# AcherStyx/SSD-Object-Detection

Hardware: AMD Instinct MI355X
Metric: images/sec SSD300 train step, batch 64 (higher is better)
Workload: dtype bf16; 1 GPU; BASELINE configs[2]: SSD300 full train step (anchor match+encode, image normalisation, conv fwd, loss, conv bwd, per-variable clip (64 variables) + Adam), per-GPU batch 64, 80 classes, synthetic COCO-shaped boxes; per_gpu_batch=64, global_batch=64, parallelism=single

## Files before the change

### include/ssd_hip.h

```cpp
#ifndef SSD_HIP_H
#define SSD_HIP_H

#include <stddef.h>
#include <stdint.h>

#ifdef __cplusplus
extern "C" {
#endif

typedef enum {
    SSD_OK = 0,
    SSD_ERR_ASSERT = -1,
    SSD_ERR_VALUE = -2,
    SSD_ERR_WORKSPACE = -3,
    SSD_ERR_LAUNCH = -4,
    SSD_ERR_UNSUPPORTED = -5
} ssd_status;

typedef enum { SSD_F32 = 0, SSD_BF16 = 1 } ssd_dtype;

int ssd_hip_abi_version(void);
const char* ssd_status_string(int status);

int ssd_priors_count(const int* grid_hw, int levels, const int* ratio_off);
// ... 271 lines not shown
    SSD_PLAN_DMA_256_256, SSD_PLAN_DMA_256_128, SSD_PLAN_DMA_256_64, SSD_PLAN_DMA_128_64, SSD_PLAN_DMA_128_128,
    SSD_PLAN_CONV0_FWD, SSD_PLAN_P512, SSD_PLAN_PW,
    SSD_PLAN_WG_FIRST = 32, SSD_PLAN_WG_PATCH_16x16, SSD_PLAN_WG_PATCH_6x40, SSD_PLAN_WG_PATCH_10x24, SSD_PLAN_WG_TILE,
    SSD_PLAN_WG_GENERIC,
    SSD_PLAN_F_FLAT = 0x100,
    SSD_PLAN_F_ROWFLAT = 0x200,
    SSD_PLAN_F_SPLITK = 0x400,
    SSD_PLAN_F_POOL_FUSED = 0x800,
    SSD_PLAN_F_S2 = 0x1000,
    SSD_PLAN_F_REDUCE_WIDE = 0x2000
};
int ssd_conv2d_fwd_plan(int B, int H, int W, int Cin, int Cout, int ksize, int stride, int pad_t, int pad_l, int Ho, int Wo,
                        int pool, size_t ws_bytes);
int ssd_conv2d_head_fwd_plan(int B, int H, int W, int Cin, int per_cell, int classes, size_t ws_bytes);
int ssd_conv2d_bwd_data_plan(int B, int H, int W, int Cin, int Cout_pad, int ksize, int stride, int pad_t, int pad_l, int Ho,
                             int Wo, int accumulate, size_t ws_bytes);
int ssd_conv2d_bwd_weight_plan(int B, int H, int W, int Cin, int Cout, int ldy, int ksize, int stride, int pad_t, int pad_l,
                               int Ho, int Wo);
const char* ssd_conv_plan_name(int plan);
int ssd_conv2d_fwd_workgroups(int B, int H, int W, int Cin, int Cout, int ksize, int stride, int pad_t, int pad_l, int Ho,
                              int Wo, int pool, size_t ws_bytes);
int ssd_conv2d_bwd_data_workgroups(int B, int H, int W, int Cin, int Cout_pad, int ksize, int stride, int pad_t, int pad_l,
                                   int Ho, int Wo, int accumulate, size_t ws_bytes);

int ssd_dev_knob(const char* name, int value);

int ssd_dev_mfma_calibration_workgroups(void);
double ssd_dev_mfma_calibration_flops(int iters);
int ssd_dev_mfma_calibration(int iters, void* stamps, void* sink, void* stream);

#ifdef __cplusplus
}
#endif
#endif
```

### ssd-object-detection_amd/csrc/conv.hip

```cpp
#include <atomic>
#include <cstdint>
#include <type_traits>
#include "common.h"
#include <hip/hip_bf16.h>
#include <stdlib.h>

#include "conv_common.h"
namespace {

template <int EPI>
__global__ void k_igemm_finalize(ConvGeom g, Epilogue ep) {
    const int n4 = (g.N + 3) >> 2;
    const long long idx = (long long)blockIdx.x * blockDim.x + threadIdx.x;
    if (idx >= (long long)g.M * n4) return;
    const int m = (int)(idx / n4), n = (int)(idx - (long long)m * n4) * 4;
    const bool full = n + 3 < g.N;
    float v[4] = {0.f, 0.f, 0.f, 0.f};
    if (full && !(g.N & 3)) {
        for (int z = 0; z < ep.ksplit; ++z) {
            const float4 t = *reinterpret_cast<const float4*>(ep.slab + ((long long)z * g.M + m) * g.N + n);
            v[0] += t.x; v[1] += t.y; v[2] += t.z; v[3] += t.w;
        }
    } else {
        for (int z = 0; z < ep.ksplit; ++z) {
// ... 390 lines not shown
        asm volatile("s_waitcnt vmcnt(6)" ::: "memory");
        SSD_PHASE_MMA(1, 0, fw0)
    }
#undef SSD_PHASE_MMA
    if (wr == 0) __builtin_amdgcn_s_barrier();

    if (staged_ok<EPI>(g, ep) && !(g.ablate & 8)) {
        asm volatile("s_waitcnt vmcnt(0)" ::: "memory");
        auto row_to_m = [&](int row) { const int m = m0 + row; return m < g.M ? m : -1; };
        staged_epilogue<EPI, 256, 256, 4, 8, 512>(acc, smem, g, ep, n0, wr * 128, wc * 64, tid, row_to_m);
        return;
    }
    int mrow[8];
#pragma unroll
    for (int p = 0; p < 8; ++p) {
        const int m = m0 + wr * 128 + p * 16 + (lane & 15);
        mrow[p] = m < g.M ? m : -1;
    }
    conv_epilogue_rows<EPI, 4, 8>(acc, g, ep, mrow, n0 + wc * 64, lane);
}

constexpr int P32_PITCH = 96;
constexpr int P32_PATCH = 32 * 1024;

template <int BN, int EPI, bool FLAT>
__global__ __launch_bounds__(512) __attribute__((amdgpu_waves_per_eu(4, 4))) void k_conv3x3_patch32(
    const bf16_raw* __restrict__ x, const bf16_raw* __restrict__ w, ConvGeom g, Epilogue ep, int tiles_x, int tiles_y, int nblocks, int rowflat) {
    constexpr int CT = BN / 32;
    constexpr int PT = 4;
    constexpr int WBYTES = BN * 64;
    constexpr int OFF_W = 2 * P32_PATCH;
    constexpr int OFF_DUMMY = OFF_W + 2 * WBYTES;
    extern __shared__ __attribute__((aligned(16))) char smem[];

    const int tid = threadIdx.x, lane = tid & 63;
    const int wave = __builtin_amdgcn_readfirstlane(tid >> 6);
    const int wave_m = wave & 3, wave_n = wave >> 2;
    const int ntn = (g.N + BN - 1) / BN;
    const int kx = blockIdx.x >> 3;
    const int pblock = (kx / ntn) * 8 + (blockIdx.x & 7);
    if (pblock >= nblocks) return;
    const int n0 = (kx % ntn) * BN;
    constexpr bool flat = FLAT;
    const int Q = FLAT ? g.W + 1 : PATCH_W;
    const int img = (g.H + 1) * Q;
    int b = 0, y0 = 0, x0 = 0, f0 = 0;
// ... 162 lines not shown
                    acc[c][p] = __builtin_amdgcn_mfma_f32_16x16x32_bf16(fw[c], fx[p], acc[c][p], 0, 0, 0);
            __builtin_amdgcn_s_setprio(3);
        }
    }
    }
    if (staged_ok<EPI>(g, ep) && !(g.ablate & 8)) {
        auto row_to_m = [&](int row) {
            if (flat) return flat_pixel(f0 + row);
            const int ir = image_row(row >> 4), xx = x0 + (row & 15);
            return (ir >= 0 && xx < g.Wo) ? ir * g.Wo + xx : -1;
        };
        auto pool_index = [&](int py, int px) -> long long {
            if (flat) return -1;
            int bb = b, gy = (y0 >> 1) + py;
            const int gx = (x0 >> 1) + px;
            if (rowflat) {
                const int R = y0 + 2 * py;
                bb = fdiv(R, g.d_h1);
                gy = (R - bb * g.d_h1.d) >> 1;
                if (bb >= g.B) return -1;
            }
            return (gy < ep.pool_h && gx < ep.pool_w) ? ((long long)bb * ep.pool_h + gy) * ep.pool_w + gx : -1;
        };
        staged_epilogue<EPI, 256, BN, CT, PT, 512>(acc, smem, g, ep, n0, wave_m * 64, wave_n * (16 * CT), tid, row_to_m, pool_index);
        return;
    }
    int mrow[PT];
#pragma unroll
    for (int p = 0; p < PT; ++p) {
        if (flat) {
            mrow[p] = flat_pixel(f0 + (4 * wave_m + p) * 16 + (lane & 15));
        } else {
            const int ir = image_row(4 * wave_m + p), xx = x0 + (lane & 15);
            mrow[p] = (ir >= 0 && xx < g.Wo) ? ir * g.Wo + xx : -1;
        }
    }
    conv_epilogue_rows<EPI, CT, PT>(acc, g, ep, mrow, n0 + wave_n * (16 * CT), lane);
}

constexpr int P5_PIX = 34 * PATCH_W;
constexpr int P5_NDMA = (P5_PIX * 6 + 63) / 64;
constexpr int P5_PATCH = P5_NDMA * 1024;
constexpr int P5_WSLOT = 128 * 64;
constexpr int P5_OFF_W = 2 * P5_PATCH;
constexpr int P5_OFF_DUMMY = P5_OFF_W + 4 * P5_WSLOT;
constexpr int P5_LDS = P5_OFF_DUMMY + 1024;

template <int EPI, bool FLAT>
__global__ __launch_bounds__(512) void k_conv3x3_p512(const bf16_raw* __restrict__ x, const bf16_raw* __restrict__ w, ConvGeom g,
                                                      Epilogue ep, int tiles_x, int tiles_y, int nblocks, int rowflat) {
    constexpr int BN = 128, CT = 4, PT = 8;
    extern __shared__ __attribute__((aligned(16))) char smem[];
    const int tid = threadIdx.x, lane = tid & 63;
    const int wave = __builtin_amdgcn_readfirstlane(tid >> 6);
    const int wave_m = wave & 3, wave_n = wave >> 2;
    const int ntn = (g.N + BN - 1) / BN;
    const int kx = blockIdx.x >> 3;
    const int pblock = (kx / ntn) * 8 + (blockIdx.x & 7);
    if (pblock >= nblocks) return;
    const int n0 = (kx % ntn) * BN;
    const int Q = FLAT ? g.W + 1 : PATCH_W;
    const int img = (g.H + 1) * Q;
    int b = 0, y0 = 0, x0 = 0, f0 = 0;
    if constexpr (FLAT) {
        f0 = pblock * 512;
    } else {
        int t = pblock;
        const int tx = t % tiles_x; t /= tiles_x;
        x0 = tx * 16;
// ... 58 lines not shown
    for (int c = 0; c < CT; ++c)
#pragma unroll
        for (int p = 0; p < PT; ++p) acc[c][p] = f32x4_t{0.f, 0.f, 0.f, 0.f};

    const int frow = lane & 15, fk = lane >> 4;
    const int xbase = (FLAT ? 8 * wave_m * 16 + frow : 8 * wave_m * PATCH_W + frow) * P32_PITCH + fk * 16;
    constexpr int prow = (FLAT ? 16 : PATCH_W) * P32_PITCH;
    int wbase;
    {
        const int row = wave_n * 64 + frow;
        wbase = P5_OFF_W + row * 64 + ((fk ^ ((-(row >> 2)) & 3)) << 4);
    }
    auto ldf = [&](int addr) { return lds_read_b128_scoped(smem + addr, smem); };
    auto load_x = [&](bf16x8_t (&fx)[PT], int pb, int tap) {
        const int tapoff = pb + xbase + ((tap / 3) * Q + tap % 3) * P32_PITCH;
#pragma unroll
        for (int p = 0; p < PT; ++p) fx[p] = ldf(tapoff + p * prow);
    };
    auto load_w = [&](bf16x8_t (&fw)[CT], int step) {
        const int wb = (step & 3) * P5_WSLOT;
#pragma unroll
        for (int c = 0; c < CT; ++c) fw[c] = ldf(wb + wbase + c * 1024);
    };
#pragma unroll
    for (int j = 0; j < 8; ++j) dma_piece(0, 0, j, true);
    dma_w(0); dma_w(1); dma_w(2);
    bf16x8_t fxa[PT], fxb[PT], fwa[CT], fwb[CT];
    asm volatile("s_waitcnt vmcnt(2)" ::: "memory");
    __builtin_amdgcn_s_barrier();
    load_x(fxa, 0, 0);
    load_w(fwa, 0);
    auto run_chunk = [&](int chunk, auto par_tag) {
        constexpr int PAR = decltype(par_tag)::value;
        const int pb = (chunk & 1) * P5_PATCH;
        const bool next_chunk = chunk + 1 < nchunk && !(g.ablate & 32);
#pragma unroll
        for (int tap = 0; tap < 9; ++tap) {
            constexpr int NT[9] = {1, 3, 5, 5, 5, 3, 1, 1, 1};
            if (NT[tap] == 1) asm volatile("s_waitcnt vmcnt(1) lgkmcnt(0)" ::: "memory");
            else if (NT[tap] == 3) asm volatile("s_waitcnt vmcnt(3) lgkmcnt(0)" ::: "memory");
            else asm volatile("s_waitcnt vmcnt(5) lgkmcnt(0)" ::: "memory");
            __builtin_amdgcn_s_barrier();
            const int step = chunk * 9 + tap;
            dma_w(step + 3);
            if (tap < 4) {
                dma_piece(chunk + 1, (chunk + 1) & 1, 2 * tap, next_chunk);
// ... 5 lines not shown
            bf16x8_t (&fwn)[CT] = ((tap + PAR) & 1) ? fwa : fwb;
            if (tap < 8) load_x(fxn, pb, tap + 1);
            else load_x(fxn, next_chunk ? (P5_PATCH - pb) : pb, next_chunk ? 0 : 8);
            load_w(fwn, step + 1 < nstep ? step + 1 : step);
#pragma unroll
            for (int c = 0; c < CT; ++c)
#pragma unroll
                for (int p = 0; p < PT; ++p)
                    acc[c][p] = __builtin_amdgcn_mfma_f32_16x16x32_bf16(fwc[c], fxc[p], acc[c][p], 0, 0, 0);
#define SSD_P5_GROUP(NM_) __builtin_amdgcn_sched_group_barrier(0x008, NM_, 0); __builtin_amdgcn_sched_group_barrier(0x100, 1, 0)
            SSD_P5_GROUP(2); SSD_P5_GROUP(2); SSD_P5_GROUP(2); SSD_P5_GROUP(2); SSD_P5_GROUP(2); SSD_P5_GROUP(2);
            SSD_P5_GROUP(2); SSD_P5_GROUP(2); SSD_P5_GROUP(2); SSD_P5_GROUP(2); SSD_P5_GROUP(2); SSD_P5_GROUP(2);
            __builtin_amdgcn_sched_group_barrier(0x008, 8, 0);
#undef SSD_P5_GROUP
            __builtin_amdgcn_sched_barrier(0);
        }
    };
    for (int chunk = 0; chunk < nchunk; chunk += 2) {
        run_chunk(chunk, std::integral_constant<int, 0>{});
        run_chunk(chunk + 1, std::integral_constant<int, 1>{});
    }
    asm volatile("s_waitcnt vmcnt(0) lgkmcnt(0)" ::: "memory");
    if (staged_ok<EPI>(g, ep)) {
        auto row_to_m = [&](int row) {
            if constexpr (FLAT) return flat_pixel(f0 + row);
            const int ir = image_row(row >> 4), xx = x0 + (row & 15);
            return (ir >= 0 && xx < g.Wo) ? ir * g.Wo + xx : -1;
        };
        auto pool_index = [&](int py, int px) -> long long {
            if (FLAT) return -1;
            int bb = b, gy = (y0 >> 1) + py;
            const int gx = (x0 >> 1) + px;
            if (rowflat) {
                const int R = y0 + 2 * py;
                bb = fdiv(R, g.d_h1);
                gy = (R - bb * g.d_h1.d) >> 1;
                if (bb >= g.B) return -1;
            }
            return (gy < ep.pool_h && gx < ep.pool_w) ? ((long long)bb * ep.pool_h + gy) * ep.pool_w + gx : -1;
        };
        staged_epilogue<EPI, 512, BN, CT, PT, 512>(acc, smem, g, ep, n0, wave_m * 128, wave_n * 64, tid, row_to_m, pool_index);
        return;
    }
    int mrow[PT];
#pragma unroll
    for (int p = 0; p < PT; ++p) {
        if constexpr (FLAT) {
            mrow[p] = flat_pixel(f0 + (8 * wave_m + p) * 16 + (lane & 15));
        } else {
            const int ir = image_row(8 * wave_m + p), xx = x0 + (lane & 15);
            mrow[p] = (ir >= 0 && xx < g.Wo) ? ir * g.Wo + xx : -1;
        }
    }
    conv_epilogue_rows<EPI, CT, PT>(acc, g, ep, mrow, n0 + wave_n * 64, lane);
}

constexpr int C64_PITCH = 160;

constexpr int C64B_ROWS = 8;
constexpr int C64B_PATCH_PIX = (C64B_ROWS + 2) * PATCH_W;
constexpr int C64B_NDMA = (C64B_PATCH_PIX * 10 + 63) / 64;
constexpr int C64B_PATCH = C64B_NDMA * 1024;
constexpr int C64B_STAGE = 2 * C64B_PATCH;
constexpr int C64B_FRAG_DEPTH = 3;
// ... 589 lines not shown
                          : (bn == 64 ? SSD_PLAN_DMA_128_64 : SSD_PLAN_DMA_128_128);
        p->flags = (p->ksplit > 1 ? SSD_PLAN_F_SPLITK : 0) | (g.s2 ? SSD_PLAN_F_S2 : 0);
        p->lds = 2 * (bm + bn) * 128;
        if (g.s2) { p->ntm = 0; for (int c = 0; c < 4; ++c) p->ntm += (unsigned)((g.cls_n[c] + bm - 1) / bm); }
    }
    p->wgs = (int)(p->ntm * p->ntn * (unsigned)p->ksplit);
    p->grid = 8 * p->ntn * ((p->ntm + 7) / 8);
    return SSD_OK;
}

template <int EPI, bool W0>
int launch_c64b(unsigned grid, int lds, const bf16_raw* x, const bf16_raw* w, const ConvGeom& g, const Epilogue& ep, int tiles_x,
                int tiles_y, const C64W0& w0, hipStream_t s) {
    auto kern = k_conv3x3_c64b<EPI, W0>;
    static OnceLds set; if (ensure_lds(set, reinterpret_cast<const void*>(kern), lds) != 0) return SSD_ERR_LAUNCH;
    hipLaunchKernelGGL(kern, dim3(grid), dim3(256), lds, s, x, w, g, ep, tiles_x, tiles_y, w0);
    return SSD_OK;
}

template <auto KERN>
int launch_patch(const IgemmPlan& p, const bf16_raw* x, const bf16_raw* w, const ConvGeom& g, const Epilogue& ep, hipStream_t s) {
    ConvGeom gk = g;
    gk.d_h1 = make_fastdiv(p.pitch);
    auto kern = KERN;
    static OnceLds set; if (ensure_lds(set, reinterpret_cast<const void*>(kern), p.lds) != 0) return SSD_ERR_LAUNCH;
    hipLaunchKernelGGL(kern, dim3(p.grid), dim3(512), p.lds, s, x, w, gk, ep, p.tiles_x, p.tiles_y, p.nblocks, p.rowflat);
    return SSD_OK;
}

template <int BM, int BN, int EPI>
int launch_dma(const IgemmPlan& p, const bf16_raw* x, const bf16_raw* w, const ConvGeom& g, const Epilogue& ep, hipStream_t s) {
    constexpr int PT = (BM == 256 && BN == 256) ? SSD_PT256 : 4;
    constexpr int NT = (BM / (16 * PT)) * (BN >= 128 ? BN / 64 : 2) * 64;
    auto kern = k_conv_igemm_dma<BM, BN, EPI, PT>;
    if (p.lds > 65536) {
        static OnceLds set; if (ensure_lds(set, reinterpret_cast<const void*>(kern), p.lds) != 0) return SSD_ERR_LAUNCH;
    }
    hipLaunchKernelGGL(kern, dim3(p.grid, (unsigned)p.ksplit), dim3(NT), p.lds, s, x, w, g, ep);
    return SSD_OK;
}

template <int EPI, int ABL>
int launch_8ph(const IgemmPlan& p, const bf16_raw* x, const bf16_raw* w, const ConvGeom& g, const Epilogue& ep, hipStream_t s) {
    auto kern = k_conv_igemm_8ph<EPI, ABL>;
    static OnceLds set; if (ensure_lds(set, reinterpret_cast<const void*>(kern), p.lds) != 0) return SSD_ERR_LAUNCH;
    hipLaunchKernelGGL(kern, dim3(p.grid), dim3(512), p.lds, s, x, w, g, ep);
// ... 73 lines not shown
    return SSD_OK;
}

int fwd_pool_geom(int B, int H, int W, int Cin, int Cout, int ksize, int stride, int pad_t, int pad_l, int Ho, int Wo, int Hp, int Wp,
                  ConvGeom* g) {
    if (Cout % 8) return SSD_ERR_VALUE;
    if ((Hp != Ho / 2 && Hp != (Ho + 1) / 2) || (Wp != Wo / 2 && Wp != (Wo + 1) / 2) || Hp <= 0 || Wp <= 0) return SSD_ERR_VALUE;
    return fwd_geom(B, H, W, Cin, Cout, ksize, stride, pad_t, pad_l, Ho, Wo, g);
}

int head_geom(int B, int H, int W, int Cin, int per_cell, int classes, ConvGeom* g) {
    const int N = per_cell * (4 + classes);
    if (!geom_ok(B, H, W, Cin, H, W, N, 3) || per_cell <= 0 || classes <= 0) return SSD_ERR_VALUE;
    *g = make_geom(B, H, W, Cin, H, W, N, 3, 3, 1, 1, 1, 1);
    return SSD_OK;
}

int bwd_data_geom(int B, int H, int W, int Cin, int Cout_pad, int ksize, int stride, int pad_t, int pad_l, int Ho, int Wo, ConvGeom* g) {
    if (!geom_ok(B, Ho, Wo, Cout_pad, H, W, Cin, ksize) || stride <= 0) return SSD_ERR_VALUE;
    *g = make_geom(B, Ho, Wo, Cout_pad, H, W, Cin, ksize, ksize, 1, stride, ksize - 1 - pad_t, ksize - 1 - pad_l);
    return SSD_OK;
}

int igemm_answer(int epi, const ConvGeom& g, const EpiArgs& ea, bool takes_pool, bool plain_fwd, size_t ws_bytes, bool want_wgs) {
    IgemmPlan p;
    const int rc = igemm_plan(epi, g, ea, takes_pool, plain_fwd, ws_bytes != 0, ws_bytes, &p);
    if (rc != SSD_OK) return rc;
    if (!want_wgs) return p.word();
    return p.wgs < 0 ? SSD_ERR_UNSUPPORTED : p.wgs;
}

}

extern "C" {

static int conv2d_fwd_impl(const void* x, const void* w, const float* bias, void* y, int B, int H, int W, int Cin, int Cout,
                           int ksize, int stride, int pad_t, int pad_l, int Ho, int Wo, int relu, void* ws, size_t ws_bytes,
                           void* stream, void* relu_bits = nullptr) {
    ConvGeom g;
    if (!x || !w || !y || fwd_geom(B, H, W, Cin, Cout, ksize, stride, pad_t, pad_l, Ho, Wo, &g) != SSD_OK) return SSD_ERR_VALUE;
    Epilogue ep = {};
    ep.bias = bias; ep.relu = relu; ep.out = static_cast<bf16_raw*>(y); ep.ldo = Cout;
    ep.relu_bits = static_cast<unsigned char*>(relu_bits);
    return launch_igemm<EPI_FWD>(x, w, g, ep, (hipStream_t)stream, ws, ws_bytes, nullptr, true);
}

int ssd_conv2d_fwd(const void* x, const void* w, const float* bias, void* y, int B, int H, int W, int Cin, int Cout,
                   int ksize, int stride, int pad_t, int pad_l, int Ho, int Wo, int relu, void* ws, size_t ws_bytes,
                   void* stream) {
    return conv2d_fwd_impl(x, w, bias, y, B, H, W, Cin, Cout, ksize, stride, pad_t, pad_l, Ho, Wo, relu, ws, ws_bytes, stream);
}
// ... 83 lines not shown

int ssd_conv2d_bwd_data_wgrad_first(const void* dy, const void* w_t, const void* relu_bits, const void* image, float* dw0,
                                    float* dbias0, int B, int H, int W, void* ws, size_t ws_bytes, void* stream) {
    if (!dy || !w_t || !relu_bits || !image || !dw0 || B <= 0 || H <= 0 || W <= 0) return SSD_ERR_VALUE;
    if (H < 16 || W < 16 || (long long)B * H * W * 64 >= (1ll << 31) - 16) return SSD_ERR_UNSUPPORTED;
    if (!ws || ws_bytes < ssd_conv2d_bwd_data_wgrad_first_workspace_bytes(B, H, W)) return SSD_ERR_WORKSPACE;
    const ConvGeom g = make_geom(B, H, W, 64, H, W, 64, 3, 3, 1, 1, 1, 1);
    Epilogue ep = {};
    ep.ldo = 64;
    ep.mask_bits = static_cast<const unsigned char*>(relu_bits);
    int tiles_x, tiles_y;
    const unsigned grid = c64b_tiling(B, H, W, 512, &tiles_x, &tiles_y);
    float* slab_w = static_cast<float*>(ws);
    float* slab_b = slab_w + (size_t)512 * 64 * 72;
    hipStream_t s = (hipStream_t)stream;
    const C64W0 w0 = {static_cast<const bf16_raw*>(image), slab_w, dbias0 ? slab_b : nullptr};
    if (launch_c64b<EPI_DGRAD, true>(grid, C64B_W0_LDS, static_cast<const bf16_raw*>(dy), static_cast<const bf16_raw*>(w_t), g, ep,
                                     tiles_x, tiles_y, w0, s) != SSD_OK || hipGetLastError() != hipSuccess)
        return SSD_ERR_LAUNCH;
    ssd_launch_wgrad_reduce(s, slab_w, 64ll * 72, 64ll * 72, dw0, slab_b, 64ll, 64, dbias0, (int)grid);
    return ssd_launch_status();
}

static int conv2d_fwd_query(bool want_wgs, int B, int H, int W, int Cin, int Cout, int ksize, int stride, int pad_t, int pad_l, int Ho,
                            int Wo, int pool, size_t ws_bytes) {
    ConvGeom g;
    EpiArgs ea = {};
    ea.out = pool != 2;
    ea.ldo = Cout;
    ea.pool_out = pool && ssd_knob("SSD_CONV_POOL_FUSE", 1);
    const int rc = pool ? fwd_pool_geom(B, H, W, Cin, Cout, ksize, stride, pad_t, pad_l, Ho, Wo, (Ho + 1) / 2, (Wo + 1) / 2, &g)
                        : fwd_geom(B, H, W, Cin, Cout, ksize, stride, pad_t, pad_l, Ho, Wo, &g);
    return rc != SSD_OK ? rc : igemm_answer(EPI_FWD, g, ea, pool != 0, pool == 0, ws_bytes, want_wgs);
}

static int conv2d_bwd_data_query(bool want_wgs, int B, int H, int W, int Cin, int Cout_pad, int ksize, int stride, int pad_t, int pad_l,
                                 int Ho, int Wo, int accumulate, size_t ws_bytes) {
    ConvGeom g;
    EpiArgs ea = {};
    ea.out = true; ea.ldo = Cin; ea.accumulate = accumulate;
    const int rc = bwd_data_geom(B, H, W, Cin, Cout_pad, ksize, stride, pad_t, pad_l, Ho, Wo, &g);
    return rc != SSD_OK ? rc : igemm_answer(EPI_DGRAD, g, ea, false, false, ws_bytes, want_wgs);
}

int ssd_conv2d_fwd_plan(int B, int H, int W, int Cin, int Cout, int ksize, int stride, int pad_t, int pad_l, int Ho, int Wo,
                        int pool, size_t ws_bytes) {
    return conv2d_fwd_query(false, B, H, W, Cin, Cout, ksize, stride, pad_t, pad_l, Ho, Wo, pool, ws_bytes);
}

int ssd_conv2d_fwd_workgroups(int B, int H, int W, int Cin, int Cout, int ksize, int stride, int pad_t, int pad_l, int Ho, int Wo,
                              int pool, size_t ws_bytes) {
    return conv2d_fwd_query(true, B, H, W, Cin, Cout, ksize, stride, pad_t, pad_l, Ho, Wo, pool, ws_bytes);
}

int ssd_conv2d_head_fwd_plan(int B, int H, int W, int Cin, int per_cell, int classes, size_t ws_bytes) {
    ConvGeom g;
    const int rc = head_geom(B, H, W, Cin, per_cell, classes, &g);
    return rc != SSD_OK ? rc : igemm_answer(EPI_HEAD, g, EpiArgs{}, false, false, ws_bytes, false);
}

int ssd_conv2d_bwd_data_plan(int B, int H, int W, int Cin, int Cout_pad, int ksize, int stride, int pad_t, int pad_l, int Ho,
                             int Wo, int accumulate, size_t ws_bytes) {
    return conv2d_bwd_data_query(false, B, H, W, Cin, Cout_pad, ksize, stride, pad_t, pad_l, Ho, Wo, accumulate, ws_bytes);
}

int ssd_conv2d_bwd_data_workgroups(int B, int H, int W, int Cin, int Cout_pad, int ksize, int stride, int pad_t, int pad_l, int Ho,
                                   int Wo, int accumulate, size_t ws_bytes) {
    return conv2d_bwd_data_query(true, B, H, W, Cin, Cout_pad, ksize, stride, pad_t, pad_l, Ho, Wo, accumulate, ws_bytes);
}

const char* ssd_conv_plan_name(int plan) {
    switch (plan & SSD_PLAN_KERNEL_MASK) {
        case SSD_PLAN_C64B: return "k_conv3x3_c64b";
        case SSD_PLAN_P32_64: return "k_conv3x3_patch32<64>";
        case SSD_PLAN_P32_128: return "k_conv3x3_patch32<128>";
        case SSD_PLAN_P512: return "k_conv3x3_p512";
        case SSD_PLAN_8PH: return "k_conv_igemm_8ph";
        case SSD_PLAN_PW: return "k_pw_gemm";
        case SSD_PLAN_DMA_256_256: return "k_conv_igemm_dma<256,256>";
        case SSD_PLAN_DMA_256_128: return "k_conv_igemm_dma<256,128>";
        case SSD_PLAN_DMA_256_64: return "k_conv_igemm_dma<256,64>";
        case SSD_PLAN_DMA_128_64: return "k_conv_igemm_dma<128,64>";
        case SSD_PLAN_DMA_128_128: return "k_conv_igemm_dma<128,128>";
        case SSD_PLAN_CONV0_FWD: return "k_conv0_fwd";
        case SSD_PLAN_WG_FIRST: return "k_conv0_wgrad";
        case SSD_PLAN_WG_PATCH_16x16: return "k_conv3x3_wgrad_patch<16,2>";
        case SSD_PLAN_WG_PATCH_6x40: return "k_conv3x3_wgrad_patch<6,5>";
        case SSD_PLAN_WG_PATCH_10x24: return "k_conv3x3_wgrad_patch<10,3>";
        case SSD_PLAN_WG_TILE: return "k_conv_wgrad_tile";
        case SSD_PLAN_WG_GENERIC: return "k_conv_wgrad";
        default: return "?";
// ... 5 lines not shown
```

### ssd-object-detection_amd/csrc/conv_common.h

```cpp
#pragma once
#include <atomic>
#include <cstdint>
#include <type_traits>
#include "common.h"
#include <hip/hip_bf16.h>

namespace {

typedef __attribute__((__vector_size__(8 * sizeof(__bf16)))) __bf16 bf16x8_t;
typedef __attribute__((__vector_size__(4 * sizeof(float)))) float f32x4_t;
typedef __attribute__((__vector_size__(4 * sizeof(short)))) short s16x4_t;
typedef unsigned short bf16_raw;

constexpr int WG = 256;

struct FastDiv {
    unsigned mg;
    int sh;
    int d;
};

inline FastDiv make_fastdiv(int d) {
    FastDiv f;
    f.d = d;
// ... 195 lines not shown
        float bias4[4];
        if constexpr (EPI == EPI_DGRAD) { bias4[0] = bias4[1] = bias4[2] = bias4[3] = 0.f; }
        else load_bias4(ep, n, g.N, full, bias4);
#pragma unroll
        for (int p = 0; p < PT; ++p) {
            const int m = mrow[p];
            if (m < 0) continue;
            float v[4] = {acc[c][p][0] + bias4[0], acc[c][p][1] + bias4[1], acc[c][p][2] + bias4[2], acc[c][p][3] + bias4[3]};
            epi_store<EPI>(v, m, n, full, g, ep);
        }
    }
}

template <int EPI>
__device__ __forceinline__ bool staged_ok(const ConvGeom& g, const Epilogue& ep) {
    if (ep.slab) return false;
    if constexpr (EPI == EPI_FWD) return (g.N & 7) == 0 && (ep.ldo & 7) == 0;
    if constexpr (EPI == EPI_DGRAD) return (g.N & 7) == 0 && (ep.ldo & 7) == 0;
    return true;
}

struct NoPool { __device__ long long operator()(int, int) const { return -1; } };

__device__ __forceinline__ uint4 lds_ld16_scoped(const char* __restrict__ p, const char* __restrict__ other) {
    (void)other;
    return *reinterpret_cast<const uint4*>(p);
}
__device__ __forceinline__ void lds_st16_scoped(char* __restrict__ p, const char* __restrict__ other, uint4 v) {
    (void)other;
    *reinterpret_cast<uint4*>(p) = v;
}
__device__ __forceinline__ void lds_st8_scoped(char* __restrict__ p, const char* __restrict__ other, uint2 v) {
    (void)other;
    *reinterpret_cast<uint2*>(p) = v;
}
__device__ __forceinline__ bf16x8_t lds_read_b128_scoped(const char* __restrict__ p, const char* __restrict__ other) {
    (void)other;
    return *reinterpret_cast<const bf16x8_t*>(p);
}
typedef __attribute__((address_space(3))) s16x4_t lds_s16x4;
__device__ __forceinline__ s16x4_t lds_read_tr16_scoped(const char* __restrict__ p, const char* __restrict__ other) {
    (void)other;
    return __builtin_amdgcn_ds_read_tr16_b64_v4i16((lds_s16x4*)p);
}

__device__ __attribute__((aligned(16))) const unsigned g_zero16[4] = {0u, 0u, 0u, 0u};

typedef __attribute__((address_space(3))) void lds_void;
typedef __attribute__((address_space(1))) const void gbl_void;

__device__ __forceinline__ void dma16_buf(__amdgpu_buffer_rsrc_t r, char* lds, unsigned off) {
    __builtin_amdgcn_raw_ptr_buffer_load_lds(r, (lds_void*)lds, 16, off, 0, 0, 0);
}

constexpr int PATCH_W = 18;
constexpr int PATCH_PIX = PATCH_W * PATCH_W;

template <int EPI, int BM, int BN, int NT, typename RowMap, typename PoolMap, bool DG_BATCHED = true>
__device__ __forceinline__ void staged_store(char* smem, const ConvGeom& g, const Epilogue& ep, int n0, int tid, RowMap row_to_m,
                                             PoolMap pool_index) {
    constexpr int CPR = BN / 8;
    if constexpr (EPI == EPI_HEAD) {
        const bool pairs = !((ep.per_cell | ep.level_off | ep.anchors_total | ep.n_loc | ep.n_conf) & 1);
        if (pairs) {
            constexpr int ITER2 = BM * BN / (2 * NT);
            for (int it = 0; it < ITER2; ++it) {
                const int idx = it * NT + tid;
                const int row = idx / (BN / 2), col = (idx - row * (BN / 2)) * 2;
                const int n = n0 + col;
                const int m = row_to_m(row);
                if (m < 0 || n >= ep.n_loc + ep.n_conf) continue;
                const unsigned val = *reinterpret_cast<const unsigned*>(smem + row * (BN * 2) + ((((col >> 3) ^ row) & (CPR - 1)) << 4) + (col & 7) * 2);
                const int b = fdiv(m, g.d_hw);
                const int pix = m - b * g.d_hw.d;
                const long long anchor0 = (long long)b * ep.anchors_total + ep.level_off + (long long)pix * ep.per_cell;
                if (n < ep.n_loc) *reinterpret_cast<unsigned*>(ep.loc + anchor0 * 4 + n) = val;
                else *reinterpret_cast<unsigned*>(ep.conf + anchor0 * ep.classes + (n - ep.n_loc)) = val;
            }
            return;
        }
        constexpr int ITER = BM * BN / NT;
        for (int it = 0; it < ITER; ++it) {
            const int idx = it * NT + tid;
            const int row = idx / BN, col = idx - row * BN;
            const int n = n0 + col;
            const int m = row_to_m(row);
            if (m < 0 || n >= ep.n_loc + ep.n_conf) continue;
            const bf16_raw val = *reinterpret_cast<const bf16_raw*>(smem + row * (BN * 2) + ((((col >> 3) ^ row) & (CPR - 1)) << 4) + (col & 7) * 2);
            const int b = fdiv(m, g.d_hw);
            const int pix = m - b * g.d_hw.d;
            const long long anchor0 = (long long)b * ep.anchors_total + ep.level_off + (long long)pix * ep.per_cell;
            if (n < ep.n_loc) ep.loc[anchor0 * 4 + n] = val;
            else ep.conf[anchor0 * ep.classes + (n - ep.n_loc)] = val;
        }
    } else {
        constexpr int ITER = BM * CPR / NT;
        const bool store_full = EPI != EPI_FWD || ep.out != nullptr;
        if constexpr (EPI == EPI_DGRAD && DG_BATCHED) {
            constexpr int DG_BATCH = ITER % 4 == 0 ? 4 : (ITER % 2 == 0 ? 2 : 1);
            const long long nb8 = g.N >> 3;
            for (int it0 = 0; it0 < ITER; it0 += DG_BATCH) {
                int mm[DG_BATCH], rr[DG_BATCH], cc[DG_BATCH];
                long long oo[DG_BATCH];
                bool ok[DG_BATCH];
#pragma unroll
                for (int j = 0; j < DG_BATCH; ++j) {
                    const int idx = (it0 + j) * NT + tid;
                    rr[j] = idx / CPR; cc[j] = idx - rr[j] * CPR;
                    const int n = n0 + cc[j] * 8;
                    mm[j] = row_to_m(rr[j]);
                    ok[j] = mm[j] >= 0 && n < g.N;
                    oo[j] = ok[j] ? (long long)mm[j] * ep.ldo + n : 0;
                }
                uint4 old[DG_BATCH], mk[DG_BATCH];
                unsigned mb[DG_BATCH], cw[DG_BATCH];
#pragma unroll
                for (int j = 0; j < DG_BATCH; ++j) { old[j] = mk[j] = make_uint4(0, 0, 0, 0); mb[j] = 0xffu; cw[j] = 0u; }
                if (ep.accumulate) {
#pragma unroll
                    for (int j = 0; j < DG_BATCH; ++j) old[j] = *reinterpret_cast<const uint4*>(ep.out + oo[j]);
                }
                if (ep.mask_src) {
#pragma unroll
                    for (int j = 0; j < DG_BATCH; ++j) mk[j] = *reinterpret_cast<const uint4*>(ep.mask_src + oo[j]);
                } else if (ep.mask_bits) {
#pragma unroll
                    for (int j = 0; j < DG_BATCH; ++j) mb[j] = ep.mask_bits[ok[j] ? (long long)mm[j] * nb8 + ((n0 >> 3) + cc[j]) : 0];
                }
                if (ep.up_code) {
#pragma unroll
                    for (int j = 0; j < DG_BATCH; ++j) cw[j] = ep.up_code[ok[j] ? (long long)mm[j] * nb8 + ((n0 >> 3) + cc[j]) : 0];
                }
#pragma unroll
                for (int j = 0; j < DG_BATCH; ++j) {
                    if (!ok[j]) continue;
                    const int row = rr[j], ch = cc[j], m = mm[j];
                    const int n = n0 + ch * 8;
                    uint4 v = lds_ld16_scoped(smem + row * (BN * 2) + (((ch ^ row) & (CPR - 1)) << 4), smem);
                    if (ep.accumulate) {
                        auto add2 = [](unsigned a, unsigned b) {
                            const float lo = __uint_as_float(a << 16) + __uint_as_float(b << 16);
                            const float hi = __uint_as_float(a & 0xffff0000u) + __uint_as_float(b & 0xffff0000u);
                            return pack_bf16x2(lo, hi);
                        };
                        v.x = add2(v.x, old[j].x); v.y = add2(v.y, old[j].y); v.z = add2(v.z, old[j].z); v.w = add2(v.w, old[j].w);
                    }
                    if (ep.mask_src) {
                        auto gate = [](unsigned val, unsigned m2) {
                            if (!(__uint_as_float(m2 << 16) > 0.f)) val &= 0xffff0000u;
                            if (!(__uint_as_float(m2 & 0xffff0000u) > 0.f)) val &= 0x0000ffffu;
                            return val;
                        };
                        v.x = gate(v.x, mk[j].x); v.y = gate(v.y, mk[j].y); v.z = gate(v.z, mk[j].z); v.w = gate(v.w, mk[j].w);
                    } else if (ep.mask_bits) {
                        v = gate_bits8(v, mb[j]);
                    }
                    if (ep.up_code) {
                        const int b = fdiv(m, g.d_hw);
                        const int rem = m - b * g.d_hw.d;
                        const int oy = fdiv(rem, g.d_w), ox = rem - oy * g.d_w.d;
                        const unsigned gw[4] = {v.x, v.y, v.z, v.w};
#pragma unroll
                        for (int q = 0; q < 4; ++q) {
                            const int iy = 2 * oy + (q >> 1), ix = 2 * ox + (q & 1);
                            if (iy >= ep.up_h || ix >= ep.up_w) continue;
                            unsigned w4[4];
#pragma unroll
                            for (int k = 0; k < 4; ++k) {
                                const unsigned lo = ((cw[j] >> (8 * k)) & 15u) == (unsigned)q ? 0x0000ffffu : 0u;
                                const unsigned hi = ((cw[j] >> (8 * k + 4)) & 15u) == (unsigned)q ? 0xffff0000u : 0u;
                                w4[k] = gw[k] & (lo | hi);
                            }
                            *reinterpret_cast<uint4*>(ep.up_out + (((long long)b * ep.up_h + iy) * ep.up_w + ix) * g.N + n) =
                                make_uint4(w4[0], w4[1], w4[2], w4[3]);
                        }
                        if (!ep.out) continue;
                    }
// ... 111 lines not shown
                            const int row = (2 * py + dy) * 16 + 2 * px + dx;
                            if (row_to_m(row) < 0) continue;
                            const uint4 v = lds_ld16_scoped(smem + row * (BN * 2) + (((ch ^ row) & (CPR - 1)) << 4), smem);
                            const unsigned wds[4] = {v.x, v.y, v.z, v.w};
#pragma unroll
                            for (int k = 0; k < 8; ++k) {
                                const float f = (k & 1) ? __uint_as_float(wds[k >> 1] & 0xffff0000u) : __uint_as_float(wds[k >> 1] << 16);
                                if (f > best[k]) { best[k] = f; pos[k] = (unsigned)(2 * dy + dx); }
                            }
                        }
                    unsigned o4[4], cw = 0;
#pragma unroll
                    for (int k = 0; k < 4; ++k) o4[k] = (__float_as_uint(best[2 * k]) >> 16) | (__float_as_uint(best[2 * k + 1]) & 0xffff0000u);
#pragma unroll
                    for (int k = 0; k < 8; ++k) cw |= (best[k] > 0.f ? pos[k] : 4u) << (4 * k);
                    *reinterpret_cast<uint4*>(ep.pool_out + po * g.N + n) = make_uint4(o4[0], o4[1], o4[2], o4[3]);
                    ep.pool_code[po * (g.N >> 3) + (n >> 3)] = cw;
                }
            }
        }
    }
}

template <int EPI, int BM, int BN, int CT, int PT, int NT, typename RowMap, typename PoolMap, bool DG_BATCHED = true>
__device__ __forceinline__ void staged_epilogue(f32x4_t (&acc)[CT][PT], char* smem, const ConvGeom& g, const Epilogue& ep,
                                                int n0, int wrow0, int wcol0, int tid, RowMap row_to_m, PoolMap pool_index) {
    constexpr int CPR = BN / 8;
    const int lane = tid & 63;
    __syncthreads();
#pragma unroll
    for (int c = 0; c < CT; ++c) {
        const int col = wcol0 + c * 16 + (lane >> 4) * 4;
        const int n = n0 + col;
        float b4[4] = {0.f, 0.f, 0.f, 0.f};
        if constexpr (EPI != EPI_DGRAD) { if (n < g.N) load_bias4(ep, n, g.N, n + 3 < g.N, b4); }
#pragma unroll
        for (int p = 0; p < PT; ++p) {
            const int row = wrow0 + p * 16 + (lane & 15);
            float v[4] = {acc[c][p][0] + b4[0], acc[c][p][1] + b4[1], acc[c][p][2] + b4[2], acc[c][p][3] + b4[3]};
            if constexpr (EPI == EPI_FWD) {
                if (ep.relu) {
#pragma unroll
                    for (int j = 0; j < 4; ++j) v[j] = fmaxf(v[j], 0.f);
                }
            }
            *reinterpret_cast<uint2*>(smem + row * (BN * 2) + ((((col >> 3) ^ row) & (CPR - 1)) << 4) + (col & 4) * 2) =
                make_uint2(pack_bf16x2(v[0], v[1]), pack_bf16x2(v[2], v[3]));
        }
    }
    __syncthreads();
    staged_store<EPI, BM, BN, NT, RowMap, PoolMap, DG_BATCHED>(smem, g, ep, n0, tid, row_to_m, pool_index);
}

template <int EPI, int BM, int BN, int CT, int PT, int NT, typename RowMap>
__device__ __forceinline__ void staged_epilogue(f32x4_t (&acc)[CT][PT], char* smem, const ConvGeom& g, const Epilogue& ep,
                                                int n0, int wrow0, int wcol0, int tid, RowMap row_to_m) {
    staged_epilogue<EPI, BM, BN, CT, PT, NT>(acc, smem, g, ep, n0, wrow0, wcol0, tid, row_to_m, NoPool{});
}

struct OnceLds { std::atomic<unsigned> done{0}; };
inline int ensure_lds(OnceLds& o, const void* fn, int bytes) {
    int dev = 0;
    if (hipGetDevice(&dev) != hipSuccess) return -1;
    const unsigned bit = 1u << (dev & 31);
    if (o.done.load(std::memory_order_acquire) & bit) return 0;
    if (hipFuncSetAttribute(fn, hipFuncAttributeMaxDynamicSharedMemorySize, bytes) != hipSuccess) return -1;
    o.done.fetch_or(bit, std::memory_order_release);
    return 0;
}

inline ConvGeom make_geom(int B, int H, int W, int C, int Ho, int Wo, int N, int KH, int KW, int mul, int div, int pad_t,
                   int pad_l) {
    ConvGeom g;
    g.B = B; g.H = H; g.W = W; g.C = C; g.Ho = Ho; g.Wo = Wo; g.N = N; g.KH = KH; g.KW = KW;
// ... 43 lines not shown
```

### ssd-object-detection_amd/csrc/knobs.hip

```cpp
#include <atomic>
#include <climits>
#include <cstring>
#include "common.h"

namespace {

struct Knob { const char* name; std::atomic<int> value; };
constexpr int KNOB_UNSET = INT_MIN;
Knob g_knobs[] = {{"SSD_ABLATE", {KNOB_UNSET}}, {"SSD_DGRAD_S2", {KNOB_UNSET}},
                  {"SSD_CONV_PATCH", {KNOB_UNSET}}, {"SSD_CONV_TILE", {KNOB_UNSET}}, {"SSD_SPLITK", {KNOB_UNSET}},
                  {"SSD_WGRAD_PATCH", {KNOB_UNSET}},
                  {"SSD_WGRAD_PATCH_SHAPE", {KNOB_UNSET}}, {"SSD_WGRAD_TILE", {KNOB_UNSET}},
                  {"SSD_CONV_PATCH_FLAT", {KNOB_UNSET}}, {"SSD_WGRAD_FIRST", {KNOB_UNSET}}, {"SSD_CONV_FIRST", {KNOB_UNSET}},
                  {"SSD_WGRAD_PATCH_XCD", {KNOB_UNSET}}, {"SSD_CONV_C64", {KNOB_UNSET}}, {"SSD_CONV_POOL_FUSE", {KNOB_UNSET}},
                  {"SSD_CONV_PATCH_ROWFLAT", {KNOB_UNSET}}, {"SSD_MATCH_FUSED", {KNOB_UNSET}}, {"SSD_CONV_P512", {KNOB_UNSET}},
                  {"SSD_C64B_WGS", {KNOB_UNSET}}, {"SSD_CONV_PW", {KNOB_UNSET}}, {"SSD_PW_WGS", {KNOB_UNSET}},
                  {"SSD_SP_ABLATE", {KNOB_UNSET}}};
Knob* find_knob(const char* name) {
    for (Knob& k : g_knobs) if (!strcmp(k.name, name)) return &k;
    return nullptr;
}

}

int ssd_knob(const char* name, int dflt) {
    Knob* k = find_knob(name);
    if (!k) return dflt;
    const int v = k->value.load(std::memory_order_relaxed);
    return v == KNOB_UNSET ? dflt : v;
}

extern "C" int ssd_dev_knob(const char* name, int value) {
    if (!name) return SSD_ERR_VALUE;
    Knob* k = find_knob(name);
    if (!k) return SSD_ERR_VALUE;
    k->value.store(value, std::memory_order_relaxed);
    return SSD_OK;
}
```

Before: 7359 images/sec.

## Prefetch epilogue row map, dgrad sign bits and bias into LDS during conv mainloop

The conv kernels now issue async buffer loads into extra LDS regions before the main loop: the dgrad ReLU-mask sign bytes and the forward bias vector for the p512 kernel. They also precompute a per-row output pixel map in LDS so the staged store reads it instead of recomputing divisions. The intent is to hide the epilogue's global mask and bias loads behind the GEMM loop and cut index arithmetic in the store phase. In exchange it raises LDS use per workgroup in p512, which can lower occupancy, and it adds a knob to turn the path off plus LDS-size query APIs.

```diff
diff --git a/include/ssd_hip.h b/include/ssd_hip.h
--- a/include/ssd_hip.h
+++ b/include/ssd_hip.h
@@ -317,6 +317,10 @@
                               int Wo, int pool, size_t ws_bytes);
 int ssd_conv2d_bwd_data_workgroups(int B, int H, int W, int Cin, int Cout_pad, int ksize, int stride, int pad_t, int pad_l,
                                    int Ho, int Wo, int accumulate, size_t ws_bytes);
+int ssd_conv2d_fwd_lds_bytes(int B, int H, int W, int Cin, int Cout, int ksize, int stride, int pad_t, int pad_l, int Ho,
+                             int Wo, int pool, size_t ws_bytes);
+int ssd_conv2d_bwd_data_lds_bytes(int B, int H, int W, int Cin, int Cout_pad, int ksize, int stride, int pad_t, int pad_l,
+                                  int Ho, int Wo, int accumulate, size_t ws_bytes);
 
 int ssd_dev_knob(const char* name, int value);
 
diff --git a/ssd-object-detection_amd/csrc/conv.hip b/ssd-object-detection_amd/csrc/conv.hip
--- a/ssd-object-detection_amd/csrc/conv.hip
+++ b/ssd-object-detection_amd/csrc/conv.hip
@@ -436,6 +436,8 @@
 
 constexpr int P32_PITCH = 96;
 constexpr int P32_PATCH = 32 * 1024;
+constexpr int EPI_NO_PREFETCH = 256;
+constexpr int P32_OFF_MAP = 2 * P32_PATCH;
 
 template <int BN, int EPI, bool FLAT>
 __global__ __launch_bounds__(512) __attribute__((amdgpu_waves_per_eu(4, 4))) void k_conv3x3_patch32(
@@ -644,7 +646,14 @@
             }
             return (gy < ep.pool_h && gx < ep.pool_w) ? ((long long)bb * ep.pool_h + gy) * ep.pool_w + gx : -1;
         };
-        staged_epilogue<EPI, 256, BN, CT, PT, 512>(acc, smem, g, ep, n0, wave_m * 64, wave_n * (16 * CT), tid, row_to_m, pool_index);
+        if constexpr (FLAT && (BN == 128 || EPI == EPI_DGRAD)) {
+            LdsSide<P32_OFF_MAP, -1, -1> side;
+            side.map = side.fill = !(g.ablate & EPI_NO_PREFETCH);
+            side.signs = side.bias = false;
+            staged_epilogue<EPI, 256, BN, CT, PT, 512>(acc, smem, g, ep, n0, wave_m * 64, wave_n * (16 * CT), tid, row_to_m, pool_index, side);
+        } else {
+            staged_epilogue<EPI, 256, BN, CT, PT, 512>(acc, smem, g, ep, n0, wave_m * 64, wave_n * (16 * CT), tid, row_to_m, pool_index);
+        }
         return;
     }
     int mrow[PT];
@@ -666,7 +675,12 @@
 constexpr int P5_WSLOT = 128 * 64;
 constexpr int P5_OFF_W = 2 * P5_PATCH;
 constexpr int P5_OFF_DUMMY = P5_OFF_W + 4 * P5_WSLOT;
-constexpr int P5_LDS = P5_OFF_DUMMY + 1024;
+constexpr int P5_LOOP_LDS = P5_OFF_DUMMY + 1024;
+constexpr int P5_OFF_SIGNS = P5_LOOP_LDS;
+constexpr int P5_OFF_MAP = P5_OFF_SIGNS + 512 * 16;
+constexpr int P5_OFF_BIAS = P5_OFF_MAP + 512 * 4;
+constexpr int P5_LDS = P5_OFF_BIAS + 128 * 4;
+static_assert(P5_LDS <= 160 * 1024, "k_conv3x3_p512: LDS of one workgroup");
 
 template <int EPI, bool FLAT>
 __global__ __launch_bounds__(512) void k_conv3x3_p512(const bf16_raw* __restrict__ x, const bf16_raw* __restrict__ w, ConvGeom g,
@@ -771,6 +785,34 @@
 #pragma unroll
         for (int c = 0; c < CT; ++c) fw[c] = ldf(wb + wbase + c * 1024);
     };
+    auto row_to_m = [&](int row) {
+        if constexpr (FLAT) return flat_pixel(f0 + row);
+        const int ir = image_row(row >> 4), xx = x0 + (row & 15);
+        return (ir >= 0 && xx < g.Wo) ? ir * g.Wo + xx : -1;
+    };
+    LdsSide<P5_OFF_MAP, P5_OFF_SIGNS, P5_OFF_BIAS> side;
+    side.map = side.fill = !(g.ablate & EPI_NO_PREFETCH) && staged_ok<EPI>(g, ep);
+    side.signs = side.bias = false;
+    if constexpr (EPI == EPI_DGRAD) {
+        const long long sign_bytes = (long long)g.M * (g.N >> 3);
+        side.signs = side.map && ep.mask_bits && !ep.mask_src && (g.N & 127) == 0 &&
+                     (reinterpret_cast<unsigned long long>(ep.mask_bits) & 15ull) == 0 && sign_bytes < (1ll << 31) - 16;
+        if (side.signs) {
+            const int m = row_to_m(tid);
+            lds_st4_scoped(smem + P5_OFF_MAP + tid * 4, smem, m);
+            side.fill = false;
+            const __amdgpu_buffer_rsrc_t sres = __builtin_amdgcn_make_buffer_rsrc((void*)ep.mask_bits, 0, (unsigned)sign_bytes, 0x00020000);
+            dma16_buf(sres, smem + P5_OFF_SIGNS + wave * 1024, m >= 0 ? (unsigned)m * (unsigned)(g.N >> 3) + (unsigned)(n0 >> 3) : OOB);
+        }
+    } else {
+        side.bias = side.map;
+        if (side.bias) {
+            const __amdgpu_buffer_rsrc_t bres = __builtin_amdgcn_make_buffer_rsrc((void*)ep.bias, 0, ep.bias ? (unsigned)g.N * 4u : 0u, 0x00020000);
+            const int n = n0 + wave * 64 + lane;
+            char* dst = wave < 2 ? smem + P5_OFF_BIAS + wave * 256 : smem + P5_OFF_DUMMY;
+            __builtin_amdgcn_raw_ptr_buffer_load_lds(bres, (lds_void*)dst, 4, (wave < 2 && n < g.N) ? (unsigned)n * 4u : OOB, 0, 0, 0);
+        }
+    }
 #pragma unroll
     for (int j = 0; j < 8; ++j) dma_piece(0, 0, j, true);
     dma_w(0); dma_w(1); dma_w(2);
@@ -822,11 +864,6 @@
     }
     asm volatile("s_waitcnt vmcnt(0) lgkmcnt(0)" ::: "memory");
     if (staged_ok<EPI>(g, ep)) {
-        auto row_to_m = [&](int row) {
-            if constexpr (FLAT) return flat_pixel(f0 + row);
-            const int ir = image_row(row >> 4), xx = x0 + (row & 15);
-            return (ir >= 0 && xx < g.Wo) ? ir * g.Wo + xx : -1;
-        };
         auto pool_index = [&](int py, int px) -> long long {
             if (FLAT) return -1;
             int bb = b, gy = (y0 >> 1) + py;
@@ -839,7 +876,7 @@
             }
             return (gy < ep.pool_h && gx < ep.pool_w) ? ((long long)bb * ep.pool_h + gy) * ep.pool_w + gx : -1;
         };
-        staged_epilogue<EPI, 512, BN, CT, PT, 512>(acc, smem, g, ep, n0, wave_m * 128, wave_n * 64, tid, row_to_m, pool_index);
+        staged_epilogue<EPI, 512, BN, CT, PT, 512>(acc, smem, g, ep, n0, wave_m * 128, wave_n * 64, tid, row_to_m, pool_index, side);
         return;
     }
     int mrow[PT];
@@ -1475,6 +1512,7 @@
 int launch_patch(const IgemmPlan& p, const bf16_raw* x, const bf16_raw* w, const ConvGeom& g, const Epilogue& ep, hipStream_t s) {
     ConvGeom gk = g;
     gk.d_h1 = make_fastdiv(p.pitch);
+    if (!ssd_knob("SSD_EPI_PREFETCH", 1)) gk.ablate |= EPI_NO_PREFETCH;
     auto kern = KERN;
     static OnceLds set; if (ensure_lds(set, reinterpret_cast<const void*>(kern), p.lds) != 0) return SSD_ERR_LAUNCH;
     hipLaunchKernelGGL(kern, dim3(p.grid), dim3(512), p.lds, s, x, w, gk, ep, p.tiles_x, p.tiles_y, p.nblocks, p.rowflat);
@@ -1594,11 +1632,12 @@
     return SSD_OK;
 }
 
-int igemm_answer(int epi, const ConvGeom& g, const EpiArgs& ea, bool takes_pool, bool plain_fwd, size_t ws_bytes, bool want_wgs) {
+int igemm_answer(int epi, const ConvGeom& g, const EpiArgs& ea, bool takes_pool, bool plain_fwd, size_t ws_bytes, int want) {
     IgemmPlan p;
     const int rc = igemm_plan(epi, g, ea, takes_pool, plain_fwd, ws_bytes != 0, ws_bytes, &p);
     if (rc != SSD_OK) return rc;
-    if (!want_wgs) return p.word();
+    if (want == 0) return p.word();
+    if (want == 2) return p.id == SSD_PLAN_PW ? SSD_ERR_UNSUPPORTED : p.lds;
     return p.wgs < 0 ? SSD_ERR_UNSUPPORTED : p.wgs;
 }
 
@@ -1728,7 +1767,7 @@
     return ssd_launch_status();
 }
 
-static int conv2d_fwd_query(bool want_wgs, int B, int H, int W, int Cin, int Cout, int ksize, int stride, int pad_t, int pad_l, int Ho,
+static int conv2d_fwd_query(int want, int B, int H, int W, int Cin, int Cout, int ksize, int stride, int pad_t, int pad_l, int Ho,
                             int Wo, int pool, size_t ws_bytes) {
     ConvGeom g;
     EpiArgs ea = {};
@@ -1737,26 +1776,26 @@
     ea.pool_out = pool && ssd_knob("SSD_CONV_POOL_FUSE", 1);
     const int rc = pool ? fwd_pool_geom(B, H, W, Cin, Cout, ksize, stride, pad_t, pad_l, Ho, Wo, (Ho + 1) / 2, (Wo + 1) / 2, &g)
                         : fwd_geom(B, H, W, Cin, Cout, ksize, stride, pad_t, pad_l, Ho, Wo, &g);
-    return rc != SSD_OK ? rc : igemm_answer(EPI_FWD, g, ea, pool != 0, pool == 0, ws_bytes, want_wgs);
-}
-
-static int conv2d_bwd_data_query(bool want_wgs, int B, int H, int W, int Cin, int Cout_pad, int ksize, int stride, int pad_t, int pad_l,
+    return rc != SSD_OK ? rc : igemm_answer(EPI_FWD, g, ea, pool != 0, pool == 0, ws_bytes, want);
+}
+
+static int conv2d_bwd_data_query(int want, int B, int H, int W, int Cin, int Cout_pad, int ksize, int stride, int pad_t, int pad_l,
                                  int Ho, int Wo, int accumulate, size_t ws_bytes) {
     ConvGeom g;
     EpiArgs ea = {};
     ea.out = true; ea.ldo = Cin; ea.accumulate = accumulate;
     const int rc = bwd_data_geom(B, H, W, Cin, Cout_pad, ksize, stride, pad_t, pad_l, Ho, Wo, &g);
-    return rc != SSD_OK ? rc : igemm_answer(EPI_DGRAD, g, ea, false, false, ws_bytes, want_wgs);
+    return rc != SSD_OK ? rc : igemm_answer(EPI_DGRAD, g, ea, false, false, ws_bytes, want);
 }
 
 int ssd_conv2d_fwd_plan(int B, int H, int W, int Cin, int Cout, int ksize, int stride, int pad_t, int pad_l, int Ho, int Wo,
                         int pool, size_t ws_bytes) {
-    return conv2d_fwd_query(false, B, H, W, Cin, Cout, ksize, stride, pad_t, pad_l, Ho, Wo, pool, ws_bytes);
+    return conv2d_fwd_query(0, B, H, W, Cin, Cout, ksize, stride, pad_t, pad_l, Ho, Wo, pool, ws_bytes);
 }
 
 int ssd_conv2d_fwd_workgroups(int B, int H, int W, int Cin, int Cout, int ksize, int stride, int pad_t, int pad_l, int Ho, int Wo,
                               int pool, size_t ws_bytes) {
-    return conv2d_fwd_query(true, B, H, W, Cin, Cout, ksize, stride, pad_t, pad_l, Ho, Wo, pool, ws_bytes);
+    return conv2d_fwd_query(1, B, H, W, Cin, Cout, ksize, stride, pad_t, pad_l, Ho, Wo, pool, ws_bytes);
 }
 
 int ssd_conv2d_head_fwd_plan(int B, int H, int W, int Cin, int per_cell, int classes, size_t ws_bytes) {
@@ -1767,12 +1806,22 @@
 
 int ssd_conv2d_bwd_data_plan(int B, int H, int W, int Cin, int Cout_pad, int ksize, int stride, int pad_t, int pad_l, int Ho,
                              int Wo, int accumulate, size_t ws_bytes) {
-    return conv2d_bwd_data_query(false, B, H, W, Cin, Cout_pad, ksize, stride, pad_t, pad_l, Ho, Wo, accumulate, ws_bytes);
+    return conv2d_bwd_data_query(0, B, H, W, Cin, Cout_pad, ksize, stride, pad_t, pad_l, Ho, Wo, accumulate, ws_bytes);
 }
 
 int ssd_conv2d_bwd_data_workgroups(int B, int H, int W, int Cin, int Cout_pad, int ksize, int stride, int pad_t, int pad_l, int Ho,
                                    int Wo, int accumulate, size_t ws_bytes) {
-    return conv2d_bwd_data_query(true, B, H, W, Cin, Cout_pad, ksize, stride, pad_t, pad_l, Ho, Wo, accumulate, ws_bytes);
+    return conv2d_bwd_data_query(1, B, H, W, Cin, Cout_pad, ksize, stride, pad_t, pad_l, Ho, Wo, accumulate, ws_bytes);
+}
+
+int ssd_conv2d_fwd_lds_bytes(int B, int H, int W, int Cin, int Cout, int ksize, int stride, int pad_t, int pad_l, int Ho, int Wo,
+                             int pool, size_t ws_bytes) {
+    return conv2d_fwd_query(2, B, H, W, Cin, Cout, ksize, stride, pad_t, pad_l, Ho, Wo, pool, ws_bytes);
+}
+
+int ssd_conv2d_bwd_data_lds_bytes(int B, int H, int W, int Cin, int Cout_pad, int ksize, int stride, int pad_t, int pad_l, int Ho,
+                                  int Wo, int accumulate, size_t ws_bytes) {
+    return conv2d_bwd_data_query(2, B, H, W, Cin, Cout_pad, ksize, stride, pad_t, pad_l, Ho, Wo, accumulate, ws_bytes);
 }
 
 const char* ssd_conv_plan_name(int plan) {
diff --git a/ssd-object-detection_amd/csrc/conv_common.h b/ssd-object-detection_amd/csrc/conv_common.h
--- a/ssd-object-detection_amd/csrc/conv_common.h
+++ b/ssd-object-detection_amd/csrc/conv_common.h
@@ -241,6 +241,19 @@
 
 struct NoPool { __device__ long long operator()(int, int) const { return -1; } };
 
+struct NoSide {
+    static constexpr int MAP_OFF = -1, SIGN_OFF = -1, BIAS_OFF = -1;
+    bool map = false, fill = false, signs = false, bias = false;
+};
+template <int MAP_OFF_, int SIGN_OFF_, int BIAS_OFF_>
+struct LdsSide {
+    static constexpr int MAP_OFF = MAP_OFF_, SIGN_OFF = SIGN_OFF_, BIAS_OFF = BIAS_OFF_;
+    bool map;
+    bool fill;
+    bool signs;
+    bool bias;
+};
+
 __device__ __forceinline__ uint4 lds_ld16_scoped(const char* __restrict__ p, const char* __restrict__ other) {
     (void)other;
     return *reinterpret_cast<const uint4*>(p);
@@ -252,6 +265,10 @@
 __device__ __forceinline__ void lds_st8_scoped(char* __restrict__ p, const char* __restrict__ other, uint2 v) {
     (void)other;
     *reinterpret_cast<uint2*>(p) = v;
+}
+__device__ __forceinline__ void lds_st4_scoped(char* __restrict__ p, const char* __restrict__ other, int v) {
+    (void)other;
+    *reinterpret_cast<int*>(p) = v;
 }
 __device__ __forceinline__ bf16x8_t lds_read_b128_scoped(const char* __restrict__ p, const char* __restrict__ other) {
     (void)other;
@@ -275,10 +292,16 @@
 constexpr int PATCH_W = 18;
 constexpr int PATCH_PIX = PATCH_W * PATCH_W;
 
-template <int EPI, int BM, int BN, int NT, typename RowMap, typename PoolMap, bool DG_BATCHED = true>
-__device__ __forceinline__ void staged_store(char* smem, const ConvGeom& g, const Epilogue& ep, int n0, int tid, RowMap row_to_m,
-                                             PoolMap pool_index) {
+template <int EPI, int BM, int BN, int NT, typename RowMap, typename PoolMap, bool DG_BATCHED = true, typename Side = NoSide>
+__device__ __forceinline__ void staged_store(char* smem, const ConvGeom& g, const Epilogue& ep, int n0, int tid, RowMap row_to_m_fn,
+                                             PoolMap pool_index, Side side = Side{}) {
     constexpr int CPR = BN / 8;
+    auto row_to_m = [&](int row) -> int {
+        if constexpr (Side::MAP_OFF >= 0) {
+            if (side.map) return *reinterpret_cast<const int*>(smem + Side::MAP_OFF + row * 4);
+        }
+        return row_to_m_fn(row);
+    };
     if constexpr (EPI == EPI_HEAD) {
         const bool pairs = !((ep.per_cell | ep.level_off | ep.anchors_total | ep.n_loc | ep.n_conf) & 1);
         if (pairs) {
@@ -318,6 +341,24 @@
         if constexpr (EPI == EPI_DGRAD && DG_BATCHED) {
             constexpr int DG_BATCH = ITER % 4 == 0 ? 4 : (ITER % 2 == 0 ? 2 : 1);
             const long long nb8 = g.N >> 3;
+            bool lds_signs = false;
+            if constexpr (Side::SIGN_OFF >= 0) {
+                static_assert(Side::SIGN_OFF < 0 || CPR == 16, "sign table: 16 bytes per tile row");
+                lds_signs = side.signs;
+            }
+            if (lds_signs && !ep.accumulate && !ep.up_code) {
+#pragma unroll 4
+                for (int it = 0; it < ITER; ++it) {
+                    const int idx = it * NT + tid;
+                    const int row = idx / CPR, ch = idx - row * CPR;
+                    const int n = n0 + ch * 8;
+                    const int m = row_to_m(row);
+                    if (m < 0 || n >= g.N) continue;
+                    const uint4 v = lds_ld16_scoped(smem + row * (BN * 2) + (((ch ^ row) & (CPR - 1)) << 4), smem);
+                    const unsigned sb = *reinterpret_cast<const unsigned char*>(smem + Side::SIGN_OFF + idx);
+                    *reinterpret_cast<uint4*>(ep.out + ((long long)m * ep.ldo + n)) = gate_bits8(v, sb);
+                }
+            } else
             for (int it0 = 0; it0 < ITER; it0 += DG_BATCH) {
                 int mm[DG_BATCH], rr[DG_BATCH], cc[DG_BATCH];
                 long long oo[DG_BATCH];
@@ -342,7 +383,7 @@
                 if (ep.mask_src) {
 #pragma unroll
                     for (int j = 0; j < DG_BATCH; ++j) mk[j] = *reinterpret_cast<const uint4*>(ep.mask_src + oo[j]);
-                } else if (ep.mask_bits) {
+                } else if (ep.mask_bits && !lds_signs) {
 #pragma unroll
                     for (int j = 0; j < DG_BATCH; ++j) mb[j] = ep.mask_bits[ok[j] ? (long long)mm[j] * nb8 + ((n0 >> 3) + cc[j]) : 0];
                 }
@@ -372,6 +413,7 @@
                         };
                         v.x = gate(v.x, mk[j].x); v.y = gate(v.y, mk[j].y); v.z = gate(v.z, mk[j].z); v.w = gate(v.w, mk[j].w);
                     } else if (ep.mask_bits) {
+                        if (lds_signs) mb[j] = *reinterpret_cast<const unsigned char*>(smem + Side::SIGN_OFF + row * CPR + ch);
                         v = gate_bits8(v, mb[j]);
                     }
                     if (ep.up_code) {
@@ -529,18 +571,31 @@
     }
 }
 
-template <int EPI, int BM, int BN, int CT, int PT, int NT, typename RowMap, typename PoolMap, bool DG_BATCHED = true>
+template <int EPI, int BM, int BN, int CT, int PT, int NT, typename RowMap, typename PoolMap, bool DG_BATCHED = true,
+          typename Side = NoSide>
 __device__ __forceinline__ void staged_epilogue(f32x4_t (&acc)[CT][PT], char* smem, const ConvGeom& g, const Epilogue& ep,
-                                                int n0, int wrow0, int wcol0, int tid, RowMap row_to_m, PoolMap pool_index) {
+                                                int n0, int wrow0, int wcol0, int tid, RowMap row_to_m, PoolMap pool_index,
+                                                Side side = Side{}) {
     constexpr int CPR = BN / 8;
     const int lane = tid & 63;
     __syncthreads();
+    if constexpr (Side::MAP_OFF >= 0) {
+        static_assert(Side::MAP_OFF < 0 || NT >= BM, "row map: one row per thread");
+        if (side.map && side.fill && tid < BM) *reinterpret_cast<int*>(smem + Side::MAP_OFF + tid * 4) = row_to_m(tid);
+    }
 #pragma unroll
     for (int c = 0; c < CT; ++c) {
         const int col = wcol0 + c * 16 + (lane >> 4) * 4;
         const int n = n0 + col;
         float b4[4] = {0.f, 0.f, 0.f, 0.f};
-        if constexpr (EPI != EPI_DGRAD) { if (n < g.N) load_bias4(ep, n, g.N, n + 3 < g.N, b4); }
+        bool lds_bias = false;
+        if constexpr (Side::BIAS_OFF >= 0) lds_bias = side.bias;
+        if constexpr (EPI != EPI_DGRAD) {
+            if (lds_bias) {
+                const float4 bv = *reinterpret_cast<const float4*>(smem + Side::BIAS_OFF + col * 4);
+                b4[0] = bv.x; b4[1] = bv.y; b4[2] = bv.z; b4[3] = bv.w;
+            } else if (n < g.N) load_bias4(ep, n, g.N, n + 3 < g.N, b4);
+        }
 #pragma unroll
         for (int p = 0; p < PT; ++p) {
             const int row = wrow0 + p * 16 + (lane & 15);
@@ -556,7 +611,7 @@
         }
     }
     __syncthreads();
-    staged_store<EPI, BM, BN, NT, RowMap, PoolMap, DG_BATCHED>(smem, g, ep, n0, tid, row_to_m, pool_index);
+    staged_store<EPI, BM, BN, NT, RowMap, PoolMap, DG_BATCHED, Side>(smem, g, ep, n0, tid, row_to_m, pool_index, side);
 }
 
 template <int EPI, int BM, int BN, int CT, int PT, int NT, typename RowMap>
diff --git a/ssd-object-detection_amd/csrc/knobs.hip b/ssd-object-detection_amd/csrc/knobs.hip
--- a/ssd-object-detection_amd/csrc/knobs.hip
+++ b/ssd-object-detection_amd/csrc/knobs.hip
@@ -15,7 +15,7 @@
                   {"SSD_WGRAD_PATCH_XCD", {KNOB_UNSET}}, {"SSD_CONV_C64", {KNOB_UNSET}}, {"SSD_CONV_POOL_FUSE", {KNOB_UNSET}},
                   {"SSD_CONV_PATCH_ROWFLAT", {KNOB_UNSET}}, {"SSD_MATCH_FUSED", {KNOB_UNSET}}, {"SSD_CONV_P512", {KNOB_UNSET}},
                   {"SSD_C64B_WGS", {KNOB_UNSET}}, {"SSD_CONV_PW", {KNOB_UNSET}}, {"SSD_PW_WGS", {KNOB_UNSET}},
-                  {"SSD_SP_ABLATE", {KNOB_UNSET}}};
+                  {"SSD_SP_ABLATE", {KNOB_UNSET}}, {"SSD_EPI_PREFETCH", {KNOB_UNSET}}};
 Knob* find_knob(const char* name) {
     for (Knob& k : g_knobs) if (!strcmp(k.name, name)) return &k;
     return nullptr;
```

Result: faster. 7465 images/sec (median of 6 runs) (+1.4%).
